# bibendovsky/oalsfxpp

Measured on AMD Instinct MI355X. Metric: Msamples/sec EAX reverb, 256-frame buffers, batch=4096; % HBM roofline, higher is better.
Workload: dtype f32

## Files before the change

### oalsfxpp_amd/csrc/hip/batch.cpp

```cpp
#include <hip/hip_runtime.h>

#include <algorithm>
#include <atomic>
#include <cstdio>
#include <chrono>
#include <cmath>
#include <cstdlib>
#include <cstring>
#include <map>
#include <mutex>
#include <new>
#include <string>
#include <type_traits>
#include <vector>

#include "../host/core.hpp"
#include "common.hpp"
#include "oalsfx_hip.h"
#include "state_io.hpp"
#include "downmix.hpp"
#include "meter.hpp"
#include "sampler.hpp"
#include "voice.hpp"
#include "oalsfx_hip_debug.h"

using namespace oalsfx_host;
using oalsfx_hip::KernelCtx;

namespace {

thread_local std::string g_last_error;

struct RingPool {
    size_t slab_floats = 0;
    std::vector<float*> free_clean;
    std::vector<float*> free_dirty;
};

struct TimedLaunch { hipEvent_t start, stop; int type; };

constexpr int kSideStreams = 3;

}

constexpr int kChainDepth = 3;
static_assert(kChainDepth >= 1 && kChainDepth <= 3, "a wavefront looks at the CUs of the two launches before it (reverb.hip, turn_cu / turn_cu2): at most three launches in flight");

struct oalsfx_batch {
    int n = 0, slots = 0, channels = 0, rate = 0, device = 0;
    int format = 0;
    DeviceDesc dev;
    std::vector<InstanceHost> inst;

    std::vector<oalsfx_slot_params> h_params;
    std::vector<oalsfx_slot_state> h_state_init;
    std::vector<oalsfx_source_params> h_source;
    std::vector<uint32_t> seq;
    std::vector<float*> h_rings;
    std::vector<size_t> ring_floats;
    bool rings_table_dirty = false;
    std::vector<uint8_t> inst_dirty;
    std::vector<int> since_update;
    std::vector<uint8_t> slot_class;
    std::vector<size_t> settling;
    std::vector<uint8_t> in_settling;
    std::vector<uint8_t> mod_ever;
    std::vector<uint8_t> xf_ok;
    int n_close[OALSFX_MAX_SLOTS] = {};
    int n_short[OALSFX_MAX_SLOTS] = {};
    bool modulated[OALSFX_MAX_SLOTS] = {};
    int n_filtered = 0;
    std::vector<uint8_t> inst_filtered;
    std::vector<int> h_lists;
    uint32_t lists_version = 0;
    uint32_t inside_version = ~0u;
    int inside_end = -1, inside_filtered = 0;
    std::vector<uint8_t> proven;
    std::vector<uint32_t> updated_gen;
    std::vector<uint32_t> inst_epoch;
    uint32_t upload_gen = 0;
    bool exact_wanted = false;
    bool exact_pending = false;
    uint32_t exact_gen = 0;
    std::vector<int> dirty_list;
    bool lists_dirty = true;
    std::vector<uint8_t> touched;
    std::vector<int> touched_list;
    std::vector<uint8_t> aux_written;

    oalsfx_slot_params* d_params = nullptr;
    oalsfx_hip::SlotStateLines* d_state = nullptr;
    oalsfx_source_params* d_source = nullptr;
    float** d_rings = nullptr;
    oalsfx_source_state* d_source_state = nullptr;
    float* d_filtered = nullptr;
    size_t filtered_capacity = 0;
    float* d_mixbuf = nullptr;
    int* d_lists = nullptr;
    int* d_lists_buf[kChainDepth + 1] = {};
    int lists_turn = 0;
    int* d_progress = nullptr;
    unsigned* d_hot = nullptr;
    unsigned* d_inst_epoch = nullptr;
    unsigned* d_exact = nullptr;
    unsigned* h_exact = nullptr;
    char fault_text[400] = {};
    long long host_prepare_ns = 0, host_stage_wait_ns = 0, host_derive_ns = 0, host_lists_ns = 0;
    unsigned* h_fault = nullptr;
    unsigned* d_fault = nullptr;
    bool chain_given_up = false;
    uint32_t gate_skew = 0;
    hipEvent_t ev_exact = nullptr;
    char* h_state_io = nullptr;
    char* d_state_io = nullptr;
    size_t state_io_capacity = 0;
    hipEvent_t ev_state_io = nullptr;
    bool state_io_pending = false;
    bool state_io_unordered = false;
    int list_offset[OALSFX_MAX_SLOTS][OALSFX_TYPE_COUNT] = {};
    int list_count[OALSFX_MAX_SLOTS][OALSFX_TYPE_COUNT] = {};
    int steady_offset[OALSFX_MAX_SLOTS] = {};
    int fast_count[OALSFX_MAX_SLOTS] = {};
    int kind_count[OALSFX_MAX_SLOTS][3] = {};
    int rest_tiles[OALSFX_MAX_SLOTS] = {};
    int fast_first[OALSFX_MAX_SLOTS] = {};
    int slow_count[OALSFX_MAX_SLOTS] = {};
    int general_offset[OALSFX_MAX_SLOTS] = {};
    int general_count[OALSFX_MAX_SLOTS] = {};
    std::map<size_t, RingPool> pools;
    std::vector<void*> chunks;
    struct RingChunk { char* base; size_t bytes; void* alloc; };
    std::vector<RingChunk> ring_chunks;
    int placed_chunks = 0, placement_candidates = 0;
    double placement_best_us = 0.0, placement_worst_us = 0.0;

    float* d_io_src = nullptr;
    float* d_io_dst = nullptr;
    size_t io_capacity = 0;
    float* h_io_src = nullptr;
    float* h_io_dst = nullptr;
    size_t h_io_capacity = 0;
    static constexpr int kPipeDepth = 3;
    struct PipeSlot { float* d_src = nullptr; float* d_dst = nullptr; hipEvent_t copied_in = nullptr, mixed = nullptr, copied_out = nullptr; bool busy = false; };
    PipeSlot pipe[kPipeDepth];
    size_t pipe_capacity = 0;
    long long pipe_turn = 0;
    hipStream_t h2d_stream = nullptr, d2h_stream = nullptr;
    int pipe_mode = 0;
    std::chrono::steady_clock::time_point pipe_probe_t0;
    double pipe_probe_us[2] = {0.0, 0.0};

    unsigned long long* d_timeline = nullptr;
    struct Stage { char* host = nullptr; char* dev = nullptr; size_t capacity = 0; hipEvent_t done = nullptr; bool pending = false; };
    Stage stage[4];
    int stage_turn = 0;
    hipEvent_t ev_uploaded = nullptr;
    hipEvent_t ev_mixed = nullptr;
    hipStream_t last_launch_stream = nullptr;
    const char* last_steady_kernel = "";
// ... 863 lines not shown
        if (name) b->last_steady_kernel = name;
        b->launched_groups += groups;
    }
    if (hand_over && count > lead) {
        ScopedTiming timing(b, OALSFX_REVERB + kTimedGeneralOffset, stream);
        oalsfx_hip::launch_reverb_general(c, slot, list + lead, count - lead, flags, stream);
    }
}

void steady_kind_counts(const oalsfx_batch* b, int slot, bool proven_usable, int counts[4])
{
    counts[0] = counts[1] = counts[2] = 0;
    counts[3] = b->slow_count[slot];
    if (proven_usable) for (int k = 0; k < 3; ++k) counts[k] = b->kind_count[slot][k];
    else counts[3] += b->fast_count[slot];
    for (int k = 0; k < 3; ++k) {
        int next = k + 1;
        while (next < 4 && counts[next] == 0) ++next;
        if (next == 4 || counts[k] == 0) continue;
        const int carry = counts[k] & 3;
        counts[k] -= carry;
        counts[next] += carry;
    }
}

int filters_inside_count(oalsfx_batch* b, int slot, const int counts[4])
{
    if (b->slots != 1 || b->channels > 2 || b->n_filtered == 0 || counts[0] + counts[1] == 0) return 0;
    const int end = counts[0] + counts[1];
    if (b->inside_version != b->lists_version || b->inside_end != end) {
        int inside = 0;
        const int* list = b->h_lists.data() + b->steady_offset[slot];
        for (int k = 0; k < end; ++k) inside += b->inst_filtered[list[k]];
        b->inside_version = b->lists_version;
        b->inside_end = end;
        b->inside_filtered = inside;
    }
    return b->inside_filtered;
}

void launch_reverb_kinds_part(oalsfx_batch* b, const KernelCtx& ctx, int slot, int flags, bool proven_usable, bool filters_inside, hipStream_t stream)
{
    int counts[4];
    steady_kind_counts(b, slot, proven_usable, counts);
    KernelCtx c = ctx;
    c.progress = nullptr;
    const bool one_kind = counts[3] == 0 && (counts[0] > 0) + (counts[1] > 0) + (counts[2] > 0) == 1;
    c.list_first = one_kind ? b->fast_first[slot] : -1;
    ScopedTiming timing(b, OALSFX_EAX_REVERB, stream);
    int groups = 0;
    const char* name = oalsfx_hip::launch_reverb_steady_kinds(c, slot, b->d_lists + b->steady_offset[slot], counts,
                                                              flags | ((debug_flags() & kDbgKernelBits) << 8) | ((debug_flags() & kDbgNoCuMajor) ? oalsfx_hip::kNoCuMajor : 0),
                                                              filters_inside, stream, &groups, slot_off_grid(b, slot));
    if (name) b->last_steady_kernel = name;
    b->launched_groups += groups;
}

void launch_reverb_pass_part(oalsfx_batch* b, const KernelCtx& ctx, int slot, int flags, const oalsfx_hip::BufferTable& table, hipStream_t stream)
{
    int counts[4];
    steady_kind_counts(b, slot, true, counts);
    ScopedTiming timing(b, OALSFX_EAX_REVERB, stream);
    int groups = 0;
    const char* name = oalsfx_hip::launch_reverb_steady_multi(ctx, slot, b->d_lists + b->steady_offset[slot], counts, table,
                                                              flags | ((debug_flags() & kDbgKernelBits) << 8) | ((debug_flags() & kDbgNoCuMajor) ? oalsfx_hip::kNoCuMajor : 0),
                                                              stream, &groups, slot_off_grid(b, slot));
    if (name) b->last_steady_kernel = name;
    b->launched_groups += groups;
}

void launch_reverb_general_part(oalsfx_batch* b, bool everything, const KernelCtx& ctx, int slot, int flags, hipStream_t stream)
{
    const int offset = everything ? b->steady_offset[slot] : b->general_offset[slot];
    const int count = b->general_count[slot] + (everything ? b->fast_count[slot] + b->slow_count[slot] : 0);
    ScopedTiming timing(b, OALSFX_REVERB + kTimedGeneralOffset, stream);
    oalsfx_hip::launch_reverb_general(ctx, slot, b->d_lists + offset, count, flags, stream);
}

bool cooperative_type(int type)
{
    return type == OALSFX_DISTORTION || type == OALSFX_ECHO || type == OALSFX_EQUALIZER || type == OALSFX_RING_MODULATOR;
}

int wave_segments(const oalsfx_batch* b, int slot, int first_type, oalsfx_hip::WaveSegments& seg)
{
    seg = oalsfx_hip::WaveSegments{};
    int n = 0, total = 0;
    auto add = [&](int count, bool coop) {
        if (count <= 0) return;
        seg.count[n] = count;
        seg.offset[n] = total;
        if (coop) seg.coop_mask |= 1u << n;
        ++n;
        total += count;
    };
    for (int t = first_type; t < OALSFX_REVERB; ++t) {
        const int count = b->list_count[slot][t];
        if (cooperative_type(t) && count >= 4) {
            add(count & ~3, true);
            add(count & 3, false);
        } else {
            add(count, false);
        }
    }
    seg.n = n;
    return total;
}

void launch_wave_group(oalsfx_batch* b, const KernelCtx& ctx, int slot, int flags, hipStream_t stream)
{
    const bool null_has_duty = (flags & (oalsfx_hip::kFirst | oalsfx_hip::kLast)) != 0;
    const int first_type = null_has_duty ? OALSFX_NULL : OALSFX_NULL + 1;
    oalsfx_hip::WaveSegments seg;
    const int count = wave_segments(b, slot, first_type, seg);
    if (count == 0) return;
    ScopedTiming timing(b, kTimedWaveEffects, stream);
    if (ctx.turn != nullptr) { flags |= (debug_flags() & kDbgHandOverBits) << 8; b->launched_groups += seg.blocks(); }
    oalsfx_hip::launch_wave_effects(ctx, slot, 1, b->d_lists + b->list_offset[slot][first_type], count, &seg, flags, stream);
}

bool mixed_grid_proven(const oalsfx_batch* b, int slot, int n)
{
    return b->slow_count[slot] == 0 && b->fast_count[slot] > 0 && (n & 63) == 0 &&
           (n - ((n - 1) / OALSFX_RV_MAX_UPDATE) * OALSFX_RV_MAX_UPDATE) / 64 >= b->rest_tiles[slot];
}

void launch_mixed_part(oalsfx_batch* b, const KernelCtx& ctx, int slot, int flags, hipStream_t stream)
{
    const bool null_has_duty = (flags & (oalsfx_hip::kFirst | oalsfx_hip::kLast)) != 0;
    const int first_type = null_has_duty ? OALSFX_NULL : OALSFX_NULL + 1;
    oalsfx_hip::WaveSegments seg;
    const int light = wave_segments(b, slot, first_type, seg);
    const int steady = b->fast_count[slot] + b->slow_count[slot];
    KernelCtx c = ctx;
    c.progress = nullptr;
    const bool proven = mixed_grid_proven(b, slot, ctx.frames);
    c.list_first = proven ? b->fast_first[slot] : -1;
    ScopedTiming timing(b, kTimedMixed, stream);
    if (ctx.turn != nullptr) flags |= (debug_flags() & kDbgKernelBits) << 8;
    int groups = 0;
    oalsfx_hip::launch_slot_mixed(c, slot, b->d_lists + b->steady_offset[slot], steady, b->d_lists + b->list_offset[slot][first_type], light,
                                  seg, flags, proven, stream, &groups);
    b->launched_groups += groups;
}

int reverb_free_run(const oalsfx_batch* b, int slot)
{
    int n = 0;
    while (slot + n < b->slots && b->list_count[slot + n][OALSFX_REVERB] + b->list_count[slot + n][OALSFX_EAX_REVERB] == 0) ++n;
    return n;
}

void poll_exact(oalsfx_batch* b)
{
    if (!b->exact_pending || hipEventQuery(b->ev_exact) != hipSuccess) return;
    b->exact_pending = false;
    const size_t total = static_cast<size_t>(b->n) * b->slots;
    for (size_t idx = 0; idx < total; ++idx) {
        if (b->proven[idx] || !b->h_exact[idx] || b->updated_gen[idx] > b->exact_gen || !reverb_settled(b, idx)) continue;
        b->proven[idx] = static_cast<uint8_t>(std::min(4u, (b->h_exact[idx] + 63u) / 64u));
        b->lists_dirty = true;
    }
}

bool check_fault(oalsfx_batch* b)
{
// ... 261 lines not shown
    ctx.source_state = b->d_source_state;
    ctx.mixbuf = b->d_mixbuf;
    ctx.timeline = b->d_timeline;
    ctx.hot = b->d_hot;
    ctx.inst_epoch = b->d_inst_epoch;
    ctx.exact = b->d_exact;
    ctx.fault = b->d_fault;
    ctx.list_first = -1;
    ctx.no_follow_up = 0;
    if (chained) {
        if (!b->chain_open) b->chain_dsts.clear();
        for (int k = 0; k < buffers; ++k) {
            const char* lo = reinterpret_cast<const char*>(dsts[k]);
            const char* hi = lo + static_cast<size_t>(b->n) * frames * b->channels * sizeof(float);
            bool known = false;
            for (auto& d : b->chain_dsts) known |= d.first <= lo && hi <= d.second;
            if (!known) b->chain_dsts.push_back({lo, hi});
        }
        if (!chain_next_launch(b, ctx, depth, &upload, &stream)) return false;
        if (!launch_params(b, upload, stream, nullptr, b->d_turn, ctx.turn_wait)) return false;
        b->chained_calls += 1;
    }
    ctx.slots = b->slots;
    ctx.channels = b->channels;
    ctx.io_stride = static_cast<long long>(frames) * b->channels;
    struct EqualPlaces {
        bool on;
        explicit EqualPlaces(bool o) : on(o) { if (on) oalsfx_hip::set_lds_per_workgroup(40960); }
        ~EqualPlaces() { if (on) oalsfx_hip::set_lds_per_workgroup(0); }
    } equal_places(chained && b->slots > 1);
    oalsfx_hip::BufferTable table{};
    if (pass) {
        for (int k = 0; k < buffers; ++k) { table.src[k] = srcs[k]; table.dst[k] = dsts[k]; }
        table.frames = frames;
        table.buffers = buffers;
    }
    for (int done = 0; done < total;) {
        const int n = std::min(total - done, OALSFX_MAX_CHUNK);
        const float* chunk_src = src + static_cast<size_t>(done) * b->channels;
        ctx.raw_src = chunk_src;
        ctx.dst = dst + static_cast<size_t>(done) * b->channels;
        ctx.frames = n;
        bool planes = filtered;
        bool filters_inside = false;
        if (filtered && b->slots == 1) {
            const SlotPlan p0 = plan_slot(b, ctx, 0, n, true);
            if (p0.by_kind && p0.steady > 0) {
                int counts[4];
                steady_kind_counts(b, 0, p0.proven_usable, counts);
                const int inside = filters_inside_count(b, 0, counts);
                if (inside > 0) {
                    filters_inside = true;
                    ctx.src_stride = static_cast<long long>(n) * b->channels;
                    planes = inside < b->n_filtered;
                    if (planes) {
                        const int before = b->steady_offset[0], behind = before + counts[0] + counts[1];
                        oalsfx_hip::launch_send_filters(ctx, chunk_src, ctx.io_stride, b->d_filtered, b->filtered_capacity, b->d_lists, before, stream);
                        oalsfx_hip::launch_send_filters(ctx, chunk_src, ctx.io_stride, b->d_filtered, b->filtered_capacity, b->d_lists + behind, b->n - behind, stream);
                    }
                }
            }
        }
        if (filters_inside) {
            ctx.src = planes ? b->d_filtered : chunk_src;
            if (!planes) ctx.src_stride = ctx.io_stride;
        } else if (filtered) {
            ctx.src_stride = static_cast<long long>(n) * b->channels;
            oalsfx_hip::launch_send_filters(ctx, chunk_src, ctx.io_stride, b->d_filtered, b->filtered_capacity, nullptr, b->n, stream);
            ctx.src = b->d_filtered;
        } else {
            ctx.src_stride = ctx.io_stride;
            ctx.src = chunk_src;
        }
        ctx.wet_plane = planes ? static_cast<long long>(b->filtered_capacity) : 0;
        for (int s = 0; s < b->slots; ++s) {
            ctx.wet_src = planes ? b->d_filtered + static_cast<size_t>(1 + s) * b->filtered_capacity : ctx.src;
            const int run = reverb_free_run(b, s);
            if (run >= 2) {
                const int run_flags = (s == 0 ? oalsfx_hip::kFirst : 0) | (s + run == b->slots ? oalsfx_hip::kLast : 0) |
                                      (planes ? oalsfx_hip::kFiltered : 0);
                {
                    ScopedTiming timing(b, kTimedWaveEffects, stream);
                    const bool grid_order = chained && s + run < b->slots;
                    const int* every = grid_order ? b->d_lists + b->steady_offset[b->slots - 1] : b->d_lists + b->list_offset[s][OALSFX_NULL];
                    oalsfx_hip::launch_wave_effects(ctx, s, run, every, b->n, nullptr,
                                                    run_flags | (chained ? ((debug_flags() & kDbgHandOverBits) | (grid_order ? 0 : 8)) << 8 : 0), stream);
                }
                if (chained) b->launched_groups = (b->n + 3) / 4;
                s += run - 1;
                continue;
            }
            if (chained && s > 0 && (!chain_launch_done(b) || !chain_next_launch(b, ctx, depth, nullptr, &stream))) return false;
            const int flags = (s == 0 ? oalsfx_hip::kFirst : 0) | (s == b->slots - 1 ? oalsfx_hip::kLast : 0) |
                              (planes ? oalsfx_hip::kFiltered : 0);
            const bool null_has_duty = (flags & (oalsfx_hip::kFirst | oalsfx_hip::kLast)) != 0;
            const SlotPlan sp = plan_slot(b, ctx, s, n, null_has_duty);
            const int light = sp.light, steady = sp.steady, reverbs = sp.reverbs;
            const bool use_steady = sp.use_steady, mixed = sp.mixed, by_kind = sp.by_kind, proven_usable = sp.proven_usable;
            bool part_on[4] = {light > 0 && !mixed, false, steady > 0, reverbs - steady > 0};
            int parts = 0;
            for (bool on : part_on) parts += on;
            const bool fork = parts > 1;
            if (fork && !b->hip_ok(hipEventRecord(b->ev_fork, stream), "hipEventRecord")) return false;
            int main_part = -1;
            for (int g = 0; g < 4; ++g)
                if (part_on[g]) main_part = (main_part < 0 || g == 3) ? g : main_part;
            int side = 0;
            for (int g = 0; g < 4; ++g) {
                if (!part_on[g]) continue;
                hipStream_t gs = stream;
                if (fork && g != main_part) {
                    gs = b->side_stream[side];
                    if (!b->hip_ok(hipStreamWaitEvent(gs, b->ev_fork, 0), "hipStreamWaitEvent")) return false;
                }
                if (g == 0) {
                    launch_wave_group(b, ctx, s, flags, gs);
                } else if (g == 2 && mixed) {
                    launch_mixed_part(b, ctx, s, flags, gs);
                } else if (g == 2 && pass) {
                    launch_reverb_pass_part(b, ctx, s, flags, table, gs);
                } else if (g == 2 && by_kind) {
                    launch_reverb_kinds_part(b, ctx, s, flags, proven_usable, filters_inside, gs);
                } else if (g == 2) {
                    launch_reverb_steady_part(b, ctx, s, flags, b->steady_offset[s], steady, sp.ragged_proven, gs);
                } else {
                    launch_reverb_general_part(b, !use_steady, ctx, s, flags, gs);
                }
                if (gs != stream) {
                    if (!b->hip_ok(hipEventRecord(b->ev_join[side], gs), "hipEventRecord")) return false;
                    ++side;
                }
            }
            for (int k = 0; k < side; ++k)
                if (!b->hip_ok(hipStreamWaitEvent(stream, b->ev_join[k], 0), "hipStreamWaitEvent")) return false;
        }
        done += n;
    }
    if (chained && !chain_launch_done(b)) return false;
    if (pass) { b->multi_buffers += buffers; b->multi_passes += 1; }
    if ((total % OALSFX_MAX_CHUNK) & 63) {
        for (size_t idx : b->settling)
            if (b->xf_ok[idx]) { b->xf_ok[idx] = 0; b->lists_dirty = true; }
    }
    advance_settling(b, total);
    b->frames_total += static_cast<uint32_t>(total);
    if (total & 31) b->off_grid_known = false;
    if (b->exact_wanted && !b->exact_pending) {
        const size_t total = static_cast<size_t>(b->n) * b->slots;
        if (!b->hip_ok(hipMemcpyAsync(b->h_exact, b->d_exact, total * sizeof(unsigned), hipMemcpyDeviceToHost, stream), "hipMemcpyAsync(exact)")) return false;
        if (!b->hip_ok(hipEventRecord(b->ev_exact, stream), "hipEventRecord")) return false;
        b->exact_pending = true;
        b->exact_wanted = false;
        b->exact_gen = b->upload_gen;
    }
    b->last_launch_stream = chained ? b->stream : stream;
    if (!chained && stream != b->stream && !b->hip_ok(hipEventRecord(b->ev_mixed, stream), "hipEventRecord")) return false;
    return b->hip_ok(hipGetLastError(), "kernel launch");
}

bool mix_device(oalsfx_batch* b, int frames, int buffers, const float* const* srcs, float* const* dsts, hipStream_t stream, bool may_chain,
                bool multi)
{
    if (b->state_io_unordered && stream != b->stream) {
        if (!b->hip_ok(hipStreamWaitEvent(stream, b->ev_state_io, 0), "hipStreamWaitEvent")) return false;
        b->state_io_unordered = false;
    }
    const int per_pass = std::max(1, OALSFX_MAX_CHUNK / std::max(frames, 1));
    const bool apart = multi && buffers_apart(b, frames, buffers, srcs, dsts);
    for (int k = 0; k < buffers;) {
// ... 1850 lines not shown
```

### oalsfxpp_amd/csrc/hip/common.hpp

```cpp
#ifndef OALSFX_HIP_COMMON_HPP
#define OALSFX_HIP_COMMON_HPP

#include <hip/hip_runtime.h>
#include <stdint.h>

#include "oalsfx_desc.h"

namespace oalsfx_hip {

struct alignas(128) SlotStateLines : oalsfx_slot_state {};
static_assert(sizeof(SlotStateLines) % 128 == 0 && sizeof(oalsfx_source_state) % 128 == 0, "an instance's records end where its cache lines end");


struct KernelCtx {
    const oalsfx_slot_params* params;
    SlotStateLines* state;
    float* const* rings;
    const oalsfx_source_params* source;
    oalsfx_source_state* source_state;
    const float* raw_src;
    const float* src;
    const float* wet_src;
    long long wet_plane;
    float* dst;
    float* mixbuf;
    int slots;
    int channels;
    int frames;
    long long io_stride;
    long long src_stride;
    int* progress;
    unsigned long long* timeline;
    unsigned* hot;
    const unsigned* inst_epoch;
    unsigned* exact;
    unsigned* fault;
    unsigned* turn;
    unsigned turn_wait;
    unsigned turn_set;
    unsigned* turn_started;
    unsigned* turn_cu;
    unsigned* turn_cu2;
    unsigned turn_two_back;
    int turn_slot;
    int list_first;
    int no_follow_up;
};

namespace hot {
enum {
    UT = 0,
    CHAIN = 128,
    MISC = 192,
    SIZE = 256,
    M_EPOCH = 0, M_OFFSET, M_EAX, M_HAS_FILTER, M_AUD_DIR, M_AUD_AUX, M_AUD_OUT, M_LATE_MASK, M_SHORT_MASK, M_MOD_F, M_MOD_INDEX, M_MOD_RANGE,
    M_MOD_DEPTH, M_MOD_COEFF, M_MOD_ON, M_SEND_MASK, M_COUNT
};
}

struct WaveSegments {
    enum { kMax = 20 };
    int n;
    unsigned coop_mask;
    int count[kMax];
    int offset[kMax];
    __host__ __device__ int blocks() const
    {
        int b = 0;
        for (int k = 0; k < n; ++k) b += (count[k] + 3) >> 2;
        return b;
    }
};

enum : int {
    kFirst = 1,
    kLast = 2,
    kNoCuMajor = 32,
    kFilterInside = 64,
    kFiltered = 16,
};

constexpr int kWave = 64;
constexpr unsigned kPlainMinTap = 192;
constexpr unsigned kPlainMinTapAhead = 224;

const char* launch_reverb_steady(const KernelCtx& ctx, int slot, const int* list, int count, int flags, bool close_taps, bool modulated,
                                 bool short_taps, bool proven, bool in_transition, hipStream_t stream, int* groups = nullptr, bool carry = false);
const char* launch_reverb_steady_kinds(const KernelCtx& ctx, int slot, const int* list, const int counts[4], int flags, bool filters_inside,
                                       hipStream_t stream, int* groups = nullptr, bool carry = false);
constexpr int kMaxPassBuffers = 32;
struct BufferTable {
    const float* src[kMaxPassBuffers];
    float* dst[kMaxPassBuffers];
    int frames;
    int buffers;
};
const char* launch_reverb_steady_multi(const KernelCtx& ctx, int slot, const int* list, const int counts[3], const BufferTable& table, int flags,
                                       hipStream_t stream, int* groups = nullptr, bool carry = false);
void launch_reverb_general(const KernelCtx& ctx, int slot, const int* list, int count, int flags, hipStream_t stream);
void launch_wave_effects(const KernelCtx& ctx, int slot, int slot_count, const int* list, int count, const WaveSegments* seg, int flags,
                         hipStream_t stream);
void launch_slot_mixed(const KernelCtx& ctx, int slot, const int* steady_list, int steady_count, const int* light_list, int light_count,
                       const WaveSegments& seg, int flags, bool proven, hipStream_t stream, int* groups = nullptr);
constexpr unsigned kFaultTurn = 1u << 12;
constexpr unsigned kFaultGate = 1u << 24;

void launch_chain_gate(const unsigned* started, unsigned target, unsigned* fault, hipStream_t stream);
void launch_send_filters(const KernelCtx& ctx, const float* src, long long src_stride, float* filtered, size_t send_floats, const int* list, int instances,
                         hipStream_t stream);
void launch_scatter_records(void* dst, size_t record_bytes, const void* packed, const int* indices, int count, hipStream_t stream);
struct ScatterJob { unsigned* dst; const unsigned* packed; const int* indices; int record_dwords; int count; int takes_turns; };
struct CopyJob { unsigned* dst; const unsigned* src; size_t dwords; int blocks; };
struct UploadJobs { ScatterJob scatter[4]; CopyJob copy[2]; const unsigned* turn; unsigned turn_wait; unsigned* fault; const unsigned* gate_started; unsigned gate_target; };
void launch_upload(UploadJobs jobs, hipStream_t stream);
void launch_null(hipStream_t stream);
void launch_fill_synthetic(float* dst, int instances, int floats_per_instance, unsigned buffer_index, hipStream_t stream);
void launch_ring_probe(float* slabs, int instances, size_t slab_floats, unsigned pos0, int waves_per_slab, hipStream_t stream);
void launch_stream_pattern(float* slabs, int instances, int dwords_per_lane, unsigned pos0, size_t slab_floats, int pos_skew, hipStream_t stream);
void launch_hbm_sweep(float* buf, size_t floats, int write, float* sink, hipStream_t stream);

void set_lds_per_workgroup(int bytes);
int lds_per_workgroup();

#if defined(__HIPCC__)

template <class K> inline int declared_lds(K kernel)
{
    hipFuncAttributes a{};
    return hipFuncGetAttributes(&a, reinterpret_cast<const void*>(kernel)) == hipSuccess ? static_cast<int>(a.sharedSizeBytes) : 0;
}

#define OALSFX_LAUNCH(kernel, grid, block, stream, ...)                                                          \
    do {                                                                                                         \
        int more_lds_ = 0;                                                                                       \
        if (oalsfx_hip::lds_per_workgroup() > 0) {                                                               \
            static const int declared_ = oalsfx_hip::declared_lds(kernel);                                       \
            more_lds_ = (declared_ > 0 && oalsfx_hip::lds_per_workgroup() > declared_) ? oalsfx_hip::lds_per_workgroup() - declared_ : 0;  \
        }                                                                                                        \
        hipLaunchKernelGGL(kernel, grid, block, more_lds_, stream, __VA_ARGS__);                                 \
    } while (0)

#define OALSFX_EQUAL_PLACES() asm volatile("" ::: "v127")

__device__ __forceinline__ int cu_major_position(int g, int total)
{
    const int base = g & ~1023;
    const int n = min(total - base, 1024), l = g - base;
    const int rounds = (n + 255) >> 8, rem = n - ((rounds - 1) << 8);
    const int c = l & 255, r = l >> 8;
    return base + (c < rem ? c * rounds + r : c * (rounds - 1) + rem + r);
}

__device__ __forceinline__ bool audible(float g) { return fabsf(g) > OALSFX_SILENCE_GAIN; }

__device__ __forceinline__ unsigned this_cu()
{
    const unsigned hw = __builtin_amdgcn_s_getreg((31 << 11) | 4), xcc = __builtin_amdgcn_s_getreg((31 << 11) | 20);
    return 0x10000u | ((xcc & 15u) << 8) | ((hw >> 8) & 0xFFu);
}

__device__ __forceinline__ bool turn_take(const KernelCtx& ctx, size_t word, int lane, int dbg, unsigned& cu_before)
{
    cu_before = 0;
    if (ctx.turn == nullptr || ctx.turn_wait == 0u) return true;
    int lost = 0;
    if (lane == 0) {
        unsigned spins = 0;
        while (__hip_atomic_load(ctx.turn + word, __ATOMIC_RELAXED, __HIP_MEMORY_SCOPE_AGENT) != ctx.turn_wait) {
            __builtin_amdgcn_s_sleep(2);
            if (++spins > (1u << 20)) {
                if (ctx.fault) __hip_atomic_fetch_add(ctx.fault, kFaultTurn, __ATOMIC_RELAXED, __HIP_MEMORY_SCOPE_SYSTEM);
                lost = 1;
                break;
            }
        }
    }
    if (__builtin_amdgcn_readfirstlane(lost)) return false;
    unsigned before_cu = 0, before_that_cu = 0;
    if (lane == 0) {
        before_cu = __hip_atomic_load(ctx.turn_cu + word, __ATOMIC_RELAXED, __HIP_MEMORY_SCOPE_AGENT);
        before_that_cu = __hip_atomic_load(ctx.turn_cu2 + word, __ATOMIC_RELAXED, __HIP_MEMORY_SCOPE_AGENT);
    }
    before_cu = __builtin_amdgcn_readfirstlane(before_cu);
    before_that_cu = __builtin_amdgcn_readfirstlane(before_that_cu);
// ... 134 lines not shown
```

### oalsfxpp_amd/csrc/hip/wave_effects.hip

```cpp
#include "wave_effects_body.hpp"

namespace oalsfx_hip {

template <int CH, bool CHN>
__global__ __launch_bounds__(256, CH == 8 ? 2 : 4) void k_wave_effects(KernelCtx ctx, int slot, int slot_count, const int* __restrict__ list, int count, WaveSegments seg,
                                                      int flags)
{
    __shared__ __attribute__((aligned(16))) float lds_all[4][wfx::kLdsFloats];
    wfx::wave_block<CH, CHN>(ctx, slot, slot_count, list, count, seg, flags, static_cast<int>(blockIdx.x), &lds_all[0][0], wfx::kLdsFloats);
    if constexpr (CH == 1) OALSFX_EQUAL_PLACES();
}

void launch_wave_effects(const KernelCtx& ctx, int slot, int slot_count, const int* list, int count, const WaveSegments* seg, int flags,
                         hipStream_t stream)
{
    if (count <= 0 || slot_count <= 0) return;
    WaveSegments s{};
    if (seg && slot_count == 1) s = *seg;
    const dim3 grid(s.n > 0 ? s.blocks() : (count + 3) / 4), block(256);
    if (ctx.turn != nullptr && ctx.channels <= 2) {
        if (ctx.channels == 1) OALSFX_LAUNCH((k_wave_effects<1, true>), grid, block, stream, ctx, slot, slot_count, list, count, s, flags);
        else OALSFX_LAUNCH((k_wave_effects<2, true>), grid, block, stream, ctx, slot, slot_count, list, count, s, flags);
        return;
    }
    if (ctx.channels == 1) OALSFX_LAUNCH((k_wave_effects<1, false>), grid, block, stream, ctx, slot, slot_count, list, count, s, flags);
    else if (ctx.channels == 2) OALSFX_LAUNCH((k_wave_effects<2, false>), grid, block, stream, ctx, slot, slot_count, list, count, s, flags);
    else OALSFX_LAUNCH((k_wave_effects<8, false>), grid, block, stream, ctx, slot, slot_count, list, count, s, flags);
}

}
```

### oalsfxpp_amd/csrc/hip/wave_effects_body.hpp

```cpp
#ifndef OALSFX_HIP_WAVE_EFFECTS_BODY_HPP
#define OALSFX_HIP_WAVE_EFFECTS_BODY_HPP

#include "common.hpp"

namespace oalsfx_hip {

namespace wfx {

constexpr int kRow = 68;
constexpr int kLdsRows = 20;
constexpr int kCoefBase = kLdsRows * kRow;
constexpr int kLdsFloats = kCoefBase + 32;

typedef __attribute__((address_space(1))) float GlobalFloat;
typedef const __attribute__((address_space(4))) oalsfx_slot_params ConstSlotParams;

struct Coef { float b0, b1, b2, a1, a2; };
template <class B> __device__ __forceinline__ Coef coef(const B& b) { return Coef{b.b0, b.b1, b.b2, b.a1, b.a2}; }

__device__ __forceinline__ void wave_sync()
{
    __builtin_amdgcn_fence(__ATOMIC_RELEASE, "wavefront");
    __builtin_amdgcn_wave_barrier();
    __builtin_amdgcn_fence(__ATOMIC_ACQUIRE, "wavefront");
// ... 614 lines not shown
    template <int CH> __device__ void tile(const Inst& I, const float* wet, float* out, int L, int Lp)
    {
        const auto& p = I.sp->u.distortion;
        const int lane = I.lane;
        float* lp = I.lds; float* sh = I.lds + kArr; float* bp = I.lds + 2 * kArr;
        const int n = 4 * L, np = 4 * Lp;
        if (L > 0) {
            const Coef c = coef(p.low_pass);
            const float X = wet[0] * 4.0F;
            const float z = 0.0F;
            const float p1 = lane == 0 ? x_hist0 : z;
            const float p2 = lane == 0 ? x_hist1 : z;
            float4 u;
            u.x = ((c.b0 * X) + (c.b1 * p1)) + (c.b2 * p2);
            u.y = ((c.b0 * z) + (c.b1 * X)) + (c.b2 * p1);
            u.z = ((c.b0 * z) + (c.b1 * z)) + (c.b2 * X);
            u.w = ((c.b0 * z) + (c.b1 * z)) + (c.b2 * z);
            *reinterpret_cast<float4*>(lp + 4 + 4 * lane) = u;
        }
        chain_phase(I, 2, [n, np](float* lds, int line) {
            float* row = lds + (line ? 2 * kArr : 0);
            const int cnt = line ? np : n;
            if (cnt == 256) chain_biquad_whole<256>(row, row[0], row[1]);
            else chain_biquad(row, 0, cnt, row[0], row[1]);
        });
        if (Lp > 0) {
            const float kept = bp[4 + 4 * lane];
#pragma unroll
            for (int c = 0; c < CH; ++c) {
                const float g = p.gains[c] * p.attenuation;
                if (c < I.channels && audible(g)) out[c] += g * kept;
            }
        }
        wave_sync();
        if (lane == 0) advance_row(bp, np);
        if (L > 0) {
            const float h2 = sh[2], h1 = sh[3];
            const float4 y = *reinterpret_cast<const float4*>(lp + 4 + 4 * lane);
            const float fc = p.edge_coeff;
            auto shape = [fc](float smp) {
                smp = (1.0F + fc) * smp / (1.0F + (fc * fabsf(smp)));
                smp = (1.0F + fc) * smp / (1.0F + (fc * fabsf(smp))) * -1.0F;
                smp = (1.0F + fc) * smp / (1.0F + (fc * fabsf(smp)));
                return smp;
            };
            const float x0 = shape(y.x), x1 = shape(y.y), x2 = shape(y.z), x3 = shape(y.w);
            float p1 = __shfl_up(x3, 1), p2 = __shfl_up(x2, 1);
            if (lane == 0) { p1 = h1; p2 = h2; }
            const Coef c = coef(p.band_pass);
            float4 u;
            u.x = ((c.b0 * x0) + (c.b1 * p1)) + (c.b2 * p2);
            u.y = ((c.b0 * x1) + (c.b1 * x0)) + (c.b2 * p1);
            u.z = ((c.b0 * x2) + (c.b1 * x1)) + (c.b2 * x0);
            u.w = ((c.b0 * x3) + (c.b1 * x2)) + (c.b2 * x1);
            *reinterpret_cast<float4*>(bp + 4 + 4 * lane) = u;
            if (lane == L - 1) { sh[2] = x2; sh[3] = x3; }
            if (lane == 0) advance_row(lp, n);
            x_hist0 = 0.0F; x_hist1 = 0.0F;
            wave_sync();
        }
    }
    __device__ void finish(const Inst& I)
    {
        if (I.lane == 0) {
            oalsfx_distortion_state& s = I.ss->u.distortion;
            const float* lp = I.lds; const float* sh = I.lds + kArr; const float* bp = I.lds + 2 * kArr;
            s.low_pass.x[0] = x_hist0; s.low_pass.x[1] = x_hist1;
            s.low_pass.y[1] = lp[2]; s.low_pass.y[0] = lp[3];
            s.band_pass.x[1] = sh[2]; s.band_pass.x[0] = sh[3];
            s.band_pass.y[1] = bp[2]; s.band_pass.y[0] = bp[3];
        }
    }
};

static_assert(3 * DistortionW::kArr <= kLdsFloats, "distortion arrays must fit the per-wave LDS");

struct Group {
    bool coop;
    int wib, duty;
    float* lds;
    int stride;
};

template <int CH, class Fx>
__device__ __forceinline__ void wave_instance(const KernelCtx& ctx, int slot, int inst, int flags, float* lds, int lane, const Group& group)
{
    const int channels = (CH == 8) ? ctx.channels : CH;
    const int frames = ctx.frames;
    const size_t sidx = static_cast<size_t>(inst) * ctx.slots + slot;
    typedef const __attribute__((address_space(4))) oalsfx_source_params ConstSourceParams;
    ConstSourceParams& SRC = *(ConstSourceParams*)(uintptr_t)(ctx.source + inst);
    const bool first = (flags & kFirst) != 0;
    const bool last = (flags & kLast) != 0;
    const bool filtered = (flags & kFiltered) != 0 && instance_has_send_filter(ctx, inst);
    const float* src = ctx.raw_src + static_cast<size_t>(inst) * ctx.io_stride;
    const float* wsrc = src;
    if (filtered) {
        src = ctx.src + static_cast<size_t>(inst) * ctx.src_stride;
        wsrc = ctx.wet_src + static_cast<size_t>(inst) * ctx.src_stride;
    }
    float* dst = ctx.dst + static_cast<size_t>(inst) * ctx.io_stride;
    float* mixbuf = ctx.mixbuf ? ctx.mixbuf + static_cast<size_t>(inst) * channels * OALSFX_MAX_CHUNK : nullptr;
    const bool send_on = SRC.aux[slot].out_channels != 0;

    Inst I;
    I.sp = (ConstSlotParams*)(uintptr_t)(ctx.params + sidx);
    I.ss = ctx.state + sidx;
    I.ring = (GlobalFloat*)(uintptr_t)ctx.rings[sidx];
    I.lds = lds;
    I.lane = lane;
    I.channels = channels;
    I.coop = group.coop;
    I.wib = group.wib;
    I.duty = group.duty;
    I.phase = 0;
    I.group_lds = group.lds;
    I.group_stride = group.stride;

    int ts_i = 0;
    auto stamp = [&]() {
        if (ctx.timeline && (inst & 63) == 0 && (inst >> 6) < 64 && lane == 0 && ts_i < 24)
            ctx.timeline[64 * 4 * 96 + (inst >> 6) * 96 + (slot & 3) * 24 + ts_i++] = clock64();
    };
    stamp();
    Fx fx;

    float n_in[CH], n_win[CH], n_mix[CH];
    auto request = [&](int base) {
        const int p = base + lane;
        const bool a = p < frames;
#pragma unroll
        for (int c = 0; c < CH; ++c) { n_in[c] = 0.0F; n_mix[c] = 0.0F; }
        if (a) {
            if (CH == 2) {
                const float2 v = *reinterpret_cast<const float2*>(src + static_cast<size_t>(p) * 2);
                n_in[0] = v.x; n_in[CH - 1] = v.y;
            } else {
#pragma unroll
                for (int c = 0; c < CH; ++c)
                    if (c < channels) n_in[c] = src[static_cast<size_t>(p) * channels + c];
            }
        }
#pragma unroll
        for (int c = 0; c < CH; ++c) n_win[c] = n_in[c];
        if (filtered && a) {
#pragma unroll
            for (int c = 0; c < CH; ++c)
                if (c < channels) n_win[c] = wsrc[static_cast<size_t>(p) * channels + c];
        }
        if (!first && a) {
#pragma unroll
            for (int c = 0; c < CH; ++c)
                if (c < channels) n_mix[c] = mixbuf[c * OALSFX_MAX_CHUNK + p];
        }
    };
    auto store_tile = [&](const float* o, int p, bool a) {
        if (!a) return;
        if (last && ctx.turn_set != 0u && CH <= 2) {
            if (CH == 2) {
                const unsigned long long both = static_cast<unsigned long long>(__float_as_uint(o[0])) | (static_cast<unsigned long long>(__float_as_uint(o[CH - 1])) << 32);
                __hip_atomic_store(reinterpret_cast<unsigned long long*>(dst + static_cast<size_t>(p) * 2), both, __ATOMIC_RELAXED, __HIP_MEMORY_SCOPE_AGENT);
            } else {
                __hip_atomic_store(reinterpret_cast<unsigned*>(dst + p), __float_as_uint(o[0]), __ATOMIC_RELAXED, __HIP_MEMORY_SCOPE_AGENT);
            }
        } else if (last) {
            if (CH == 2) {
                *reinterpret_cast<float2*>(dst + static_cast<size_t>(p) * 2) = make_float2(o[0], o[CH - 1]);
            } else {
#pragma unroll
                for (int c = 0; c < CH; ++c)
                    if (c < channels) dst[static_cast<size_t>(p) * channels + c] = o[c];
            }
        } else {
#pragma unroll
            for (int c = 0; c < CH; ++c)
                if (c < channels) mixbuf[c * OALSFX_MAX_CHUNK + p] = o[c];
        }
    };
    constexpr int kLag = LagOf<Fx>::value;
    float held[CH];
    int held_pos = 0, held_L = 0;
#pragma unroll
    for (int c = 0; c < CH; ++c) held[c] = 0.0F;
    request(0);
    fx.init(I);
    stamp();
    for (int base = 0; base < frames + (kLag ? 64 : 0); base += 64) {
        const int L = base < frames ? min(64, frames - base) : 0;
        const bool act = lane < L;
        const int pos = base + lane;
        float in[CH], win[CH], out[CH];
#pragma unroll
        for (int c = 0; c < CH; ++c) { in[c] = n_in[c]; win[c] = n_win[c]; out[c] = 0.0F; }
        float mix[CH];
#pragma unroll
        for (int c = 0; c < CH; ++c) mix[c] = n_mix[c];
        if (base + 64 < frames) request(base + 64);
        __builtin_amdgcn_sched_barrier(0);
        float wet[4] = {0.0F, 0.0F, 0.0F, 0.0F};
#pragma unroll
        for (int c = 0; c < CH; ++c) {
            if (c >= channels) continue;
            if (first) {
#pragma unroll
                for (int o = 0; o < CH; ++o) {
                    const float g = SRC.direct.gains[c][o];
                    if (o < channels && audible(g)) out[o] += in[c] * g;
                }
            }
            if (send_on) {
#pragma unroll
                for (int k = 0; k < 4; ++k) {
                    const float g = SRC.aux[slot].gains[c][k];
                    if (audible(g)) wet[k] += win[c] * g;
                }
            }
        }
        if (!first) {
#pragma unroll
            for (int c = 0; c < CH; ++c) out[c] = mix[c];
        }
        stamp();
        if constexpr (kLag != 0) {
            fx.template tile<CH>(I, wet, held, L, held_L);
            stamp();
            store_tile(held, held_pos, lane < held_L);
#pragma unroll
            for (int c = 0; c < CH; ++c) held[c] = out[c];
            held_pos = pos;
            held_L = L;
        } else {
            fx.template tile<CH>(I, wet, out, L);
            stamp();
            store_tile(out, pos, act);
        }
    }

    fx.finish(I);
    if (lane == 0) I.ss->seen_seq = I.sp->update_seq;
    if (first && !filtered && lane < channels) send_history_follow(ctx, inst, lane, channels, frames, src);
}


template <int CH>
__device__ __forceinline__ void wave_slots(const KernelCtx& ctx, int slot, int slot_count, int inst, int flags, float* lds, int lane, const Group& group)
{
    for (int sl = slot; sl < slot + slot_count; ++sl) {
        const int f = (flags & kFiltered) | ((flags & kFirst) && sl == slot ? kFirst : 0) | ((flags & kLast) && sl == slot + slot_count - 1 ? kLast : 0);
        const int type = __builtin_amdgcn_readfirstlane(ctx.params[static_cast<size_t>(inst) * ctx.slots + sl].type);
        KernelCtx c = ctx;
        c.wet_src = ctx.wet_src + static_cast<size_t>(sl - slot) * ctx.wet_plane;
        switch (type) {
        case OALSFX_NULL:
            if (f & (kFirst | kLast)) wave_instance<CH, NullW>(c, sl, inst, f, lds, lane, group);
            break;
        case OALSFX_CHORUS:
        case OALSFX_FLANGER: wave_instance<CH, ModDelayW>(c, sl, inst, f, lds, lane, group); break;
        case OALSFX_COMPRESSOR: wave_instance<CH, CompressorW>(c, sl, inst, f, lds, lane, group); break;
        case OALSFX_DEDICATED_DIALOG:
        case OALSFX_DEDICATED_LFE: wave_instance<CH, DedicatedW>(c, sl, inst, f, lds, lane, group); break;
        case OALSFX_DISTORTION: wave_instance<CH, DistortionW>(c, sl, inst, f, lds, lane, group); break;
        case OALSFX_ECHO: wave_instance<CH, EchoW>(c, sl, inst, f, lds, lane, group); break;
        case OALSFX_EQUALIZER: wave_instance<CH, EqualizerW>(c, sl, inst, f, lds, lane, group); break;
        case OALSFX_RING_MODULATOR: wave_instance<CH, RingModW>(c, sl, inst, f, lds, lane, group); break;
        default: break;
        }
        wave_sync();
    }
}

template <int CH, bool CHN = false>
__device__ __forceinline__ void wave_block(const KernelCtx& ctx, int slot, int slot_count, const int* __restrict__ list, int count,
                                           const WaveSegments& seg, int flags, int block, float* lds_group, int lds_stride)
{
    const int lane = threadIdx.x & 63;
    const int wib = __builtin_amdgcn_readfirstlane(threadIdx.x >> 6);
    if (CHN && ctx.turn_started != nullptr && threadIdx.x == 0) __hip_atomic_fetch_add(ctx.turn_started, 1u, __ATOMIC_RELAXED, __HIP_MEMORY_SCOPE_AGENT);
    Group group{false, wib, block & 3, lds_group, lds_stride};
    int w = block * 4 + wib;
    if (seg.n > 0) {
        int k = 0, first_block = 0;
        for (; k + 1 < seg.n; ++k) {
            const int b = (seg.count[k] + 3) >> 2;
            if (block < first_block + b) break;
            first_block += b;
        }
        const int local = (block - first_block) * 4 + wib;
        group.coop = ((seg.coop_mask >> k) & 1u) != 0;
        if (local >= seg.count[k]) return;
        w = seg.offset[k] + local;
    } else {
        if (CHN && !((flags >> 8) & 8)) w = cu_major_position(block, (count + 3) >> 2) * 4 + wib;
        if (w >= count) return;
    }
    const int inst = __builtin_amdgcn_readfirstlane(list[w]);
    unsigned cu_before = 0;
    const size_t word = static_cast<size_t>(inst) * ctx.slots + ctx.turn_slot;
    if (CHN && ((flags >> 8) & 4) && ctx.turn != nullptr && ctx.turn_wait != 0u) {
        unsigned junk = 0;
        for (int sl = slot; sl < slot + slot_count; ++sl) {
            const unsigned* st = reinterpret_cast<const unsigned*>(ctx.state + static_cast<size_t>(inst) * ctx.slots + sl);
#pragma unroll
            for (int k = 0; k < static_cast<int>(sizeof(SlotStateLines) / 256); ++k) {
                unsigned a;
                asm volatile("global_load_dword %0, %1, off\n\ts_waitcnt vmcnt(0)" : "=v"(a) : "v"(st + 64 * k + lane) : "memory");
                junk ^= a;
            }
        }
        if (ctx.mixbuf != nullptr) {
            const unsigned* mb = reinterpret_cast<const unsigned*>(ctx.mixbuf + static_cast<size_t>(inst) * ctx.channels * OALSFX_MAX_CHUNK);
            for (int c = 0; c < ctx.channels; ++c) {
                unsigned a;
                asm volatile("global_load_dword %0, %1, off\n\ts_waitcnt vmcnt(0)" : "=v"(a) : "v"(mb + c * OALSFX_MAX_CHUNK + 32 * lane) : "memory");
                junk ^= a;
            }
        }
        if (junk == 0x7E57AB1Eu && ctx.timeline) ctx.timeline[0] = junk;
    }
    const bool mine = !CHN || turn_take(ctx, word, lane, flags >> 8, cu_before);
    if (CHN && group.coop) { if (__syncthreads_or(mine ? 0 : 1)) return; }
    else if (!mine) return;
    wave_slots<CH>(ctx, slot, slot_count, inst, flags, lds_group + wib * lds_stride, lane, group);
    if (CHN) turn_hand_on(ctx, word, lane, cu_before);
}

}

}

#endif
```

Measured before the change: 25690.

## Add run kernel with per-slot cooperative groups and deferred send-history follow

Adds a k_wave_run kernel for mono and stereo batches that processes a run of consecutive slots per instance. For each slot it decides cooperatively whether all four wavefronts in a block share the same effect type, using host-computed RunHints (cached per list version) plus an LDS check. This enables cooperative processing per slot instead of only per segment. It also captures the last two raw frames up front and performs send-history follow once after the whole run. The cost is extra LDS barriers, a host scan over the lists, and a larger LDS footprint when chained.

```diff
diff --git a/oalsfxpp_amd/csrc/hip/batch.cpp b/oalsfxpp_amd/csrc/hip/batch.cpp
--- a/oalsfxpp_amd/csrc/hip/batch.cpp
+++ b/oalsfxpp_amd/csrc/hip/batch.cpp
@@ -75,6 +75,9 @@
     uint32_t lists_version = 0;
     uint32_t inside_version = ~0u;
     int inside_end = -1, inside_filtered = 0;
+    uint32_t run_version = ~0u;
+    int run_list = -1, run_slot = -1, run_slots = 0;
+    oalsfx_hip::RunHints run_cached{};
     std::vector<uint8_t> proven;
     std::vector<uint32_t> updated_gen;
     std::vector<uint32_t> inst_epoch;
@@ -1104,6 +1107,45 @@
     return type == OALSFX_DISTORTION || type == OALSFX_ECHO || type == OALSFX_EQUALIZER || type == OALSFX_RING_MODULATOR;
 }
 
+bool run_shares_type(int type)
+{
+    return cooperative_type(type) && type != OALSFX_ECHO;
+}
+
+const oalsfx_hip::RunHints& run_hints(oalsfx_batch* b, int list, int s, int run)
+{
+    if (b->run_version == b->lists_version && b->run_list == list && b->run_slot == s && b->run_slots == run) return b->run_cached;
+    oalsfx_hip::RunHints h{};
+    const int groups = b->n / 4;
+    unsigned before = 0;
+    for (int g = 0; g < groups; ++g) {
+        const int* e = b->h_lists.data() + list + 4 * g;
+        unsigned mask = 0;
+        for (int k = 0; k < run; ++k) {
+            const int t = b->h_params[static_cast<size_t>(e[0]) * b->slots + s + k].type;
+            bool same = run_shares_type(t);
+            for (int w = 1; w < 4 && same; ++w) same = b->h_params[static_cast<size_t>(e[w]) * b->slots + s + k].type == t;
+            if (same) mask |= 1u << k;
+        }
+        if (mask != 0 && mask == before) {
+            h.count[h.n - 1] += 1;
+        } else if (mask != 0) {
+            if (h.n == oalsfx_hip::RunHints::kMax) break;
+            h.first[h.n] = g;
+            h.count[h.n] = 1;
+            h.slots[h.n] = mask;
+            h.n += 1;
+        }
+        before = mask;
+    }
+    b->run_version = b->lists_version;
+    b->run_list = list;
+    b->run_slot = s;
+    b->run_slots = run;
+    b->run_cached = h;
+    return b->run_cached;
+}
+
 int wave_segments(const oalsfx_batch* b, int slot, int first_type, oalsfx_hip::WaveSegments& seg)
 {
     seg = oalsfx_hip::WaveSegments{};
@@ -1531,9 +1573,11 @@
                 {
                     ScopedTiming timing(b, kTimedWaveEffects, stream);
                     const bool grid_order = chained && s + run < b->slots;
-                    const int* every = grid_order ? b->d_lists + b->steady_offset[b->slots - 1] : b->d_lists + b->list_offset[s][OALSFX_NULL];
-                    oalsfx_hip::launch_wave_effects(ctx, s, run, every, b->n, nullptr,
-                                                    run_flags | (chained ? ((debug_flags() & kDbgHandOverBits) | (grid_order ? 0 : 8)) << 8 : 0), stream);
+                    const int every_at = grid_order ? b->steady_offset[b->slots - 1] : b->list_offset[s][OALSFX_NULL];
+                    const int* every = b->d_lists + every_at;
+                    const int wave_flags = run_flags | (chained ? ((debug_flags() & kDbgHandOverBits) | (grid_order ? 0 : 8)) << 8 : 0);
+                    if (b->channels <= 2) oalsfx_hip::launch_wave_run(ctx, s, run, every, b->n, run_hints(b, every_at, s, run), wave_flags, stream);
+                    else oalsfx_hip::launch_wave_effects(ctx, s, run, every, b->n, nullptr, wave_flags, stream);
                 }
                 if (chained) b->launched_groups = (b->n + 3) / 4;
                 s += run - 1;
diff --git a/oalsfxpp_amd/csrc/hip/common.hpp b/oalsfxpp_amd/csrc/hip/common.hpp
--- a/oalsfxpp_amd/csrc/hip/common.hpp
+++ b/oalsfxpp_amd/csrc/hip/common.hpp
@@ -72,6 +72,14 @@
     }
 };
 
+struct RunHints {
+    enum { kMax = 8 };
+    int n;
+    int first[kMax];
+    int count[kMax];
+    unsigned slots[kMax];
+};
+
 enum : int {
     kFirst = 1,
     kLast = 2,
@@ -100,6 +108,8 @@
 void launch_reverb_general(const KernelCtx& ctx, int slot, const int* list, int count, int flags, hipStream_t stream);
 void launch_wave_effects(const KernelCtx& ctx, int slot, int slot_count, const int* list, int count, const WaveSegments* seg, int flags,
                          hipStream_t stream);
+void launch_wave_run(const KernelCtx& ctx, int slot, int slot_count, const int* list, int count, const RunHints& hints, int flags,
+                     hipStream_t stream);
 void launch_slot_mixed(const KernelCtx& ctx, int slot, const int* steady_list, int steady_count, const int* light_list, int light_count,
                        const WaveSegments& seg, int flags, bool proven, hipStream_t stream, int* groups = nullptr);
 constexpr unsigned kFaultTurn = 1u << 12;
diff --git a/oalsfxpp_amd/csrc/hip/wave_effects.hip b/oalsfxpp_amd/csrc/hip/wave_effects.hip
--- a/oalsfxpp_amd/csrc/hip/wave_effects.hip
+++ b/oalsfxpp_amd/csrc/hip/wave_effects.hip
@@ -9,6 +9,30 @@
     __shared__ __attribute__((aligned(16))) float lds_all[4][wfx::kLdsFloats];
     wfx::wave_block<CH, CHN>(ctx, slot, slot_count, list, count, seg, flags, static_cast<int>(blockIdx.x), &lds_all[0][0], wfx::kLdsFloats);
     if constexpr (CH == 1) OALSFX_EQUAL_PLACES();
+}
+
+template <int CH, bool CHN>
+__global__ __launch_bounds__(256, 4) void k_wave_run(KernelCtx ctx, int slot, int slot_count, const int* __restrict__ list, int count, RunHints hints, int flags)
+{
+    constexpr int kStride = CHN ? (40960 - 256) / 16 : wfx::kLdsFloats;
+    static_assert(kStride >= wfx::kLdsFloats && kStride % 4 == 0, "a wavefront's rows, 16-byte aligned");
+    __shared__ __attribute__((aligned(16))) float lds_all[4][kStride];
+    wfx::wave_block<CH, CHN, true>(ctx, slot, slot_count, list, count, WaveSegments{}, flags, static_cast<int>(blockIdx.x), &lds_all[0][0], kStride, &hints);
+    OALSFX_EQUAL_PLACES();
+}
+
+void launch_wave_run(const KernelCtx& ctx, int slot, int slot_count, const int* list, int count, const RunHints& hints, int flags, hipStream_t stream)
+{
+    if (count <= 0 || slot_count <= 0) return;
+    const dim3 grid((count + 3) / 4), block(256);
+    const bool chained = ctx.turn != nullptr;
+    if (ctx.channels == 1) {
+        if (chained) OALSFX_LAUNCH((k_wave_run<1, true>), grid, block, stream, ctx, slot, slot_count, list, count, hints, flags);
+        else OALSFX_LAUNCH((k_wave_run<1, false>), grid, block, stream, ctx, slot, slot_count, list, count, hints, flags);
+    } else {
+        if (chained) OALSFX_LAUNCH((k_wave_run<2, true>), grid, block, stream, ctx, slot, slot_count, list, count, hints, flags);
+        else OALSFX_LAUNCH((k_wave_run<2, false>), grid, block, stream, ctx, slot, slot_count, list, count, hints, flags);
+    }
 }
 
 void launch_wave_effects(const KernelCtx& ctx, int slot, int slot_count, const int* list, int count, const WaveSegments* seg, int flags,
diff --git a/oalsfxpp_amd/csrc/hip/wave_effects_body.hpp b/oalsfxpp_amd/csrc/hip/wave_effects_body.hpp
--- a/oalsfxpp_amd/csrc/hip/wave_effects_body.hpp
+++ b/oalsfxpp_amd/csrc/hip/wave_effects_body.hpp
@@ -720,7 +720,7 @@
     int stride;
 };
 
-template <int CH, class Fx>
+template <int CH, class Fx, bool FOLLOW = true>
 __device__ __forceinline__ void wave_instance(const KernelCtx& ctx, int slot, int inst, int flags, float* lds, int lane, const Group& group)
 {
     const int channels = (CH == 8) ? ctx.channels : CH;
@@ -876,7 +876,9 @@
 
     fx.finish(I);
     if (lane == 0) I.ss->seen_seq = I.sp->update_seq;
-    if (first && !filtered && lane < channels) send_history_follow(ctx, inst, lane, channels, frames, src);
+    if constexpr (FOLLOW) {
+        if (first && !filtered && lane < channels) send_history_follow(ctx, inst, lane, channels, frames, src);
+    }
 }
 
 
@@ -907,16 +909,89 @@
     }
 }
 
-template <int CH, bool CHN = false>
+__device__ __forceinline__ bool run_shares_type(int type)
+{
+    return type == OALSFX_DISTORTION || type == OALSFX_EQUALIZER || type == OALSFX_RING_MODULATOR;
+}
+
+template <int CH>
+__device__ __forceinline__ void run_slots(const KernelCtx& ctx, int slot, int slot_count, int inst, int flags, float* lds, int lane, const Group& group,
+                                          unsigned coop_slots)
+{
+    const bool follow = (flags & kFirst) && !((flags & kFiltered) && instance_has_send_filter(ctx, inst)) && lane < CH;
+    const float* raw = ctx.raw_src + static_cast<size_t>(inst) * ctx.io_stride;
+    float newest = 0.0F, older = 0.0F;
+    if (follow && ctx.frames >= 2) {
+        newest = raw[static_cast<size_t>(ctx.frames - 1) * CH + lane];
+        older = raw[static_cast<size_t>(ctx.frames - 2) * CH + lane];
+    }
+    for (int sl = slot; sl < slot + slot_count; ++sl) {
+        const int f = (flags & kFiltered) | ((flags & kFirst) && sl == slot ? kFirst : 0) | ((flags & kLast) && sl == slot + slot_count - 1 ? kLast : 0);
+        const int type = __builtin_amdgcn_readfirstlane(ctx.params[static_cast<size_t>(inst) * ctx.slots + sl].type);
+        KernelCtx c = ctx;
+        c.wet_src = ctx.wet_src + static_cast<size_t>(sl - slot) * ctx.wet_plane;
+        Group g = group;
+        g.coop = false;
+        if ((coop_slots >> (sl - slot)) & 1u) {
+            constexpr int kPost = kCoefBase + 31;
+            if (lane == 0) reinterpret_cast<int*>(lds)[kPost] = type;
+            lds_barrier();
+            int same = 1;
+#pragma unroll
+            for (int k = 0; k < 4; ++k) same &= reinterpret_cast<const int*>(group.lds + k * group.stride)[kPost] == type ? 1 : 0;
+            lds_barrier();
+            g.coop = __builtin_amdgcn_readfirstlane(same) != 0 && run_shares_type(type);
+        }
+        switch (type) {
+        case OALSFX_NULL:
+            if (f & (kFirst | kLast)) wave_instance<CH, NullW, false>(c, sl, inst, f, lds, lane, g);
+            break;
+        case OALSFX_CHORUS:
+        case OALSFX_FLANGER: wave_instance<CH, ModDelayW, false>(c, sl, inst, f, lds, lane, g); break;
+        case OALSFX_COMPRESSOR: wave_instance<CH, CompressorW, false>(c, sl, inst, f, lds, lane, g); break;
+        case OALSFX_DEDICATED_DIALOG:
+        case OALSFX_DEDICATED_LFE: wave_instance<CH, DedicatedW, false>(c, sl, inst, f, lds, lane, g); break;
+        case OALSFX_DISTORTION: wave_instance<CH, DistortionW, false>(c, sl, inst, f, lds, lane, g); break;
+        case OALSFX_ECHO: wave_instance<CH, EchoW, false>(c, sl, inst, f, lds, lane, g); break;
+        case OALSFX_EQUALIZER: wave_instance<CH, EqualizerW, false>(c, sl, inst, f, lds, lane, g); break;
+        case OALSFX_RING_MODULATOR: wave_instance<CH, RingModW, false>(c, sl, inst, f, lds, lane, g); break;
+        default: break;
+        }
+        wave_sync();
+    }
+    if (follow) {
+        if (ctx.frames >= 2) {
+            unsigned sends = 1u;
+            for (int s = 0; s < ctx.slots; ++s)
+                if (ctx.source[inst].aux[s].out_channels != 0) sends |= 2u << s;
+            send_history_follow_values(ctx, inst, lane, sends, newest, older);
+        } else {
+            send_history_follow(ctx, inst, lane, CH, ctx.frames, raw);
+        }
+    }
+}
+
+template <int CH, bool CHN = false, bool RUN = false>
 __device__ __forceinline__ void wave_block(const KernelCtx& ctx, int slot, int slot_count, const int* __restrict__ list, int count,
-                                           const WaveSegments& seg, int flags, int block, float* lds_group, int lds_stride)
-{
+                                           const WaveSegments& seg, int flags, int block, float* lds_group, int lds_stride,
+                                           const RunHints* hints = nullptr)
+{
+    static_assert(!RUN || CH <= 2, "multichannel runs stay on k_wave_effects");
     const int lane = threadIdx.x & 63;
     const int wib = __builtin_amdgcn_readfirstlane(threadIdx.x >> 6);
     if (CHN && ctx.turn_started != nullptr && threadIdx.x == 0) __hip_atomic_fetch_add(ctx.turn_started, 1u, __ATOMIC_RELAXED, __HIP_MEMORY_SCOPE_AGENT);
     Group group{false, wib, block & 3, lds_group, lds_stride};
     int w = block * 4 + wib;
-    if (seg.n > 0) {
+    unsigned coop_slots = 0;
+    if constexpr (RUN) {
+        int g = block;
+        if (CHN && !((flags >> 8) & 8)) g = cu_major_position(block, (count + 3) >> 2);
+        for (int k = 0; k < hints->n; ++k)
+            if (g >= hints->first[k] && g - hints->first[k] < hints->count[k]) coop_slots = hints->slots[k];
+        if (g * 4 + 4 > count) coop_slots = 0;
+        w = g * 4 + wib;
+        if (w >= count) return;
+    } else if (seg.n > 0) {
         int k = 0, first_block = 0;
         for (; k + 1 < seg.n; ++k) {
             const int b = (seg.count[k] + 3) >> 2;
@@ -956,9 +1031,10 @@
         if (junk == 0x7E57AB1Eu && ctx.timeline) ctx.timeline[0] = junk;
     }
     const bool mine = !CHN || turn_take(ctx, word, lane, flags >> 8, cu_before);
-    if (CHN && group.coop) { if (__syncthreads_or(mine ? 0 : 1)) return; }
+    if (CHN && (group.coop || (RUN && coop_slots != 0u))) { if (__syncthreads_or(mine ? 0 : 1)) return; }
     else if (!mine) return;
-    wave_slots<CH>(ctx, slot, slot_count, inst, flags, lds_group + wib * lds_stride, lane, group);
+    if constexpr (RUN) run_slots<CH>(ctx, slot, slot_count, inst, flags, lds_group + wib * lds_stride, lane, group, coop_slots);
+    else wave_slots<CH>(ctx, slot, slot_count, inst, flags, lds_group + wib * lds_stride, lane, group);
     if (CHN) turn_hand_on(ctx, word, lane, cu_before);
 }
 
```

After: 25940, median of 2. About the same (+1.0%).
